# TuringLang/Bijectors.jl

Measured on NVIDIA H100. Metric: samples/sec: with_logabsdet_jacobian through 8-layer Planar flow, D=128, higher is better.
Workload: dtype f32

## Files before the change

bijectors.jl_b200/csrc/b2b_chain_v1.cu:

```cuda
#include "b2b_chain_v1_prog.cuh"

namespace b2b {

template <int D, int TPC, int CPT, int NW>
__global__ void __launch_bounds__(NW * 32, 1)
    chain_v1_kernel(const __grid_constant__ B2BChainParams P, const __grid_constant__ V1Extra E,
                    const __grid_constant__ CUtensorMap map_x, const __grid_constant__ CUtensorMap map_y) {
  const InterpProg<D, TPC, CPT> prog{P};
  v1_run<D, TPC, CPT, NW>(P, E, map_x, map_y, prog);
}

typedef void (*v1_kernel_t)(const B2BChainParams, const V1Extra, const CUtensorMap, const CUtensorMap);

struct V1Plan : V1Geom {
  v1_kernel_t kernel;
  int shape;
};

static int plan_v1(B2BChainParams& p, V1Plan& plan) {
  const int D = p.D;
  if (!(D == 32 || D == 64 || D == 128 || D == 256)) return B2B_EUNSUPPORTED;
  if (v1_check_io(p) != 0) return B2B_EUNSUPPORTED;
  int off = 0;
  for (int l = 0; l < p.L; ++l) {
    const int k = p.layers[l].kind;
    if (k == B2B_PERMUTE || k == B2B_COUPLING_AFFINE) return B2B_EUNSUPPORTED;
    p.soff[l] = off;
    off += (b2b_layer_smem_floats(p.layers[l], D) + 3) & ~3;
  }
  p.scratch_off = -1;
  bool per_row = false;
  for (int l = 0; l < p.L; ++l) per_row |= p.layers[l].kind == B2B_RQS || p.layers[l].kind == B2B_STACKED_EW;
  static const int cfg = getenv("B2B_V1_CFG") ? atoi(getenv("B2B_V1_CFG")) : 0;
  int nw, tpc, cpt = 1;
  if (D == 256) { plan.kernel = chain_v1_kernel<256, 4, 1, 12>; nw = 12; tpc = 4; }
  else if (D == 128) {
    if (cfg == 2218 && !per_row) { plan.kernel = chain_v1_kernel<128, 2, 2, 8>; nw = 8; tpc = 2; cpt = 2; }
    else if (cfg == 2112 || per_row) { plan.kernel = chain_v1_kernel<128, 2, 1, 12>; nw = 12; tpc = 2; }
    else { plan.kernel = chain_v1_kernel<128, 1, 1, 8>; nw = 8; tpc = 1; }
  }
  else if (D == 64) {
    if (cfg == 1128 && !per_row) { plan.kernel = chain_v1_kernel<64, 1, 2, 8>; nw = 8; tpc = 1; cpt = 2; }
    else { plan.kernel = chain_v1_kernel<64, 1, 1, 12>; nw = 12; tpc = 1; }
  }
  else { plan.kernel = chain_v1_kernel<32, 1, 1, 16>; nw = 16; tpc = 1; }
  plan.shape = D * 10000 + tpc * 1000 + cpt * 100 + nw;
  return v1_geometry(D, p.N, nw, (32 / tpc) * cpt, (size_t)off, plan);
}

}

int b2b_v1_plan(B2BChainParams& p, b2b::V1Geom& g, int* shape) {
  b2b::V1Plan plan;
  const int rc = b2b::plan_v1(p, plan);
  if (rc != 0) return rc;
  g = plan;
  *shape = plan.shape;
  return 0;
}

int b2b_chain_grid_size_v1(const B2BChainParams& p) {
  B2BChainParams q = p;
  b2b::V1Plan plan;
  if (b2b::plan_v1(q, plan) != 0) return 0;
  return plan.grid;
}

int b2b_launch_chain_v1(const B2BChainParams& p, cudaStream_t stream) {
  using namespace b2b;
  B2BChainParams q = p;
  V1Plan plan;
  const int rc = plan_v1(q, plan);
  if (rc != 0) return rc;
  CUtensorMap mx, my;
  if (!make_maps(q, plan.cols, &mx, &my, &plan.extra.tma3d)) return B2B_EUNSUPPORTED;
  cudaError_t e = cudaFuncSetAttribute(plan.kernel, cudaFuncAttributeMaxDynamicSharedMemorySize, (int)plan.smem);
  if (e != cudaSuccess) return (int)e;
  plan.kernel<<<plan.grid, plan.nw * 32, plan.smem, stream>>>(q, plan.extra, mx, my);
  return (int)cudaGetLastError();
}
```

bijectors.jl_b200/csrc/b2b_planar_const.cu:

```cuda
#include "b2b_planar_common.cuh"

namespace b2b {

template <int D>
struct PlanarHP {
  float v[2 * HP_MAX_L * D + 2 * HP_MAX_L];
};

template <int D>
struct ArgSrc {
  static constexpr bool kDerive = false;
  const PlanarHP<D>& H;
  int invmask;
  __device__ __forceinline__ bool inv(int l) const { return (invmask >> l) & 1; }
};

struct DevSrc {
  static constexpr bool kDerive = true;
  int invmask;
  __device__ __forceinline__ bool inv(int l) const { return (invmask >> l) & 1; }
};

template <int D, int DIR, bool MVN, class Src>
struct PlanarProg {
// ... 40 lines not shown
        acc[(i & 1) * 2 + 0] = b2b_ffma2(make_float2(w.x, w.y), x[0][2 * i], acc[(i & 1) * 2 + 0]);
        acc[(i & 1) * 2 + 1] = b2b_ffma2(make_float2(w.z, w.w), x[0][2 * i + 1], acc[(i & 1) * 2 + 1]);
      }
      const float2 s = b2b_fadd2(b2b_fadd2(acc[0], acc[1]), b2b_fadd2(acc[2], acc[3]));
      const float wz = s.x + s.y;
      const float cc_ = cb[l], bb = cb[L + l];
      float t, s2;
      if (DIR == 0 || (DIR == 2 && !src.inv(l))) {
        tanh_sech2(wz + bb, t, s2);
        lj[0] += log1pf(cc_ * s2);
      } else {
        if constexpr (TAB) find_alpha_tab(wz, cc_, bb, tab + l * PT_FLOATS, t, s2);
        else find_alpha_ts(wz, cc_, bb, t, s2);
        lj[0] -= log1pf(cc_ * s2);
        t = -t;
      }
      const float2 t2 = make_float2(t, t);
#pragma unroll
      for (int i = 0; i < D / 4; ++i) {
        const float4 u = u4[i];
        x[0][2 * i] = b2b_ffma2(make_float2(u.x, u.y), t2, x[0][2 * i]);
        x[0][2 * i + 1] = b2b_ffma2(make_float2(u.z, u.w), t2, x[0][2 * i + 1]);
      }
    }
    if (MVN) mvnormal_apply<D, 1, 1>(x, ctx, params + mvn_off(), lj);
  }
};

template <int D, int NW, int DIR>
__global__ void __launch_bounds__(NW * 32, 1)
    planar_arg_kernel(const __grid_constant__ B2BChainParams P, const __grid_constant__ V1Extra E,
                      const __grid_constant__ CUtensorMap map_x, const __grid_constant__ CUtensorMap map_y,
                      const __grid_constant__ PlanarHP<D> H, const int L, const int invmask) {
  const PlanarProg<D, DIR, false, ArgSrc<D>> prog{{H, invmask}, P, L};
  v1_run<D, 1, 1, NW>(P, E, map_x, map_y, prog);
}

template <int D, int NW, int DIR, bool MVN>
__global__ void __launch_bounds__(NW * 32, 1)
    planar_dev_kernel(const __grid_constant__ B2BChainParams P, const __grid_constant__ V1Extra E,
                      const __grid_constant__ CUtensorMap map_x, const __grid_constant__ CUtensorMap map_y,
                      const int L, const int invmask) {
  const PlanarProg<D, DIR, MVN, DevSrc> prog{{invmask}, P, L};
  v1_run<D, 1, 1, NW>(P, E, map_x, map_y, prog);
}

template <int D, int NW, int DIR>
static int launch_arg(const B2BChainParams& q, const V1Geom& g, const CUtensorMap& mx, const CUtensorMap& my, int L,
                      const float* packed, int invmask, cudaStream_t stream) {
  static PlanarHP<D> H;
  static std::mutex mu;
  std::lock_guard<std::mutex> lock(mu);
  memcpy(H.v, packed, sizeof(float) * (size_t)(2 * L * D + 2 * L));
  auto kernel = planar_arg_kernel<D, NW, DIR>;
  cudaError_t e = cudaFuncSetAttribute(kernel, cudaFuncAttributeMaxDynamicSharedMemorySize, (int)g.smem);
  if (e != cudaSuccess) return (int)e;
  kernel<<<g.grid, NW * 32, g.smem, stream>>>(q, g.extra, mx, my, H, L, invmask);
  return (int)cudaGetLastError();
}

template <int D, int NW, int DIR, bool MVN = false>
static int launch_dev(const B2BChainParams& q, const V1Geom& g, const CUtensorMap& mx, const CUtensorMap& my, int L,
                      int invmask, cudaStream_t stream) {
  auto kernel = planar_dev_kernel<D, NW, DIR, MVN>;
  cudaError_t e = cudaFuncSetAttribute(kernel, cudaFuncAttributeMaxDynamicSharedMemorySize, (int)g.smem);
  if (e != cudaSuccess) return (int)e;
  kernel<<<g.grid, NW * 32, g.smem, stream>>>(q, g.extra, mx, my, L, invmask);
  return (int)cudaGetLastError();
}

template <int D, int NW>
static int dispatch(int L, const B2BChainParams& q, const V1Geom& g, const CUtensorMap& mx, const CUtensorMap& my,
                    const float* packed, int invmask, bool mvn, cudaStream_t stream) {
  const int all = (1 << L) - 1;
  const int dir = (invmask & all) == 0 ? 0 : ((invmask & all) == all ? 1 : 2);
  if (packed) {
    if (dir == 0) return launch_arg<D, NW, 0>(q, g, mx, my, L, packed, invmask, stream);
    if (dir == 1) return launch_arg<D, NW, 1>(q, g, mx, my, L, packed, invmask, stream);
    return launch_arg<D, NW, 2>(q, g, mx, my, L, packed, invmask, stream);
  }
  if (mvn) {
    if (dir == 1) return launch_dev<D, NW, 1, true>(q, g, mx, my, L, invmask, stream);
    return B2B_EUNSUPPORTED;
  }
  if (dir == 0) return launch_dev<D, NW, 0>(q, g, mx, my, L, invmask, stream);
  if (dir == 1) return launch_dev<D, NW, 1>(q, g, mx, my, L, invmask, stream);
  return launch_dev<D, NW, 2>(q, g, mx, my, L, invmask, stream);
}

static int launch_planar(const B2BChainParams& p, int L, const float* packed, int invmask, bool mvn,
                                  cudaStream_t stream) {
  B2BChainParams q = p;
  q.scratch_off = -1;
  if (!(q.D == 32 || q.D == 64 || q.D == 128) || L < 1 || L > HP_MAX_L) return B2B_EUNSUPPORTED;
  if (v1_check_io(q) != 0) return B2B_EUNSUPPORTED;
  V1Geom g;
  const size_t pf = (size_t)((2 * L * q.D + 2 * L + 3) & ~3) + (mvn ? 2 * q.D + 4 : 0) +
                    ((!packed && invmask != 0) ? (size_t)L * PT_FLOATS : 0);
  const int rc = v1_geometry(q.D, q.N, hp_warps(q.D), 32, pf, g);
  if (rc != 0) return rc;
  CUtensorMap mx, my;
  if (!make_maps(q, g.cols, &mx, &my, &g.extra.tma3d)) return B2B_EUNSUPPORTED;
  if (q.D == 128) return dispatch<128, 8>(L, q, g, mx, my, packed, invmask, mvn, stream);
  if (q.D == 64) return dispatch<64, 12>(L, q, g, mx, my, packed, invmask, mvn, stream);
  return dispatch<32, 16>(L, q, g, mx, my, packed, invmask, mvn, stream);
}

}

int b2b_planar_const_grid_size(const B2BChainParams& p) {
  using namespace b2b;
  if (!(p.D == 32 || p.D == 64 || p.D == 128)) return 0;
  V1Geom g;
  if (v1_geometry(p.D, p.N, hp_warps(p.D), 32, 0, g) != 0) return 0;
  return g.grid;
}

int b2b_launch_planar_hostparams(const B2BChainParams& p, int L, const float* packed, int invmask,
                                 cudaStream_t stream) {
  return b2b::launch_planar(p, L, packed, invmask, false, stream);
}
// ... 25 lines not shown
```

bijectors.jl_b200/csrc/b2b_planar_vjp.cu:

```cuda
#include "b2b_planar_common.cuh"

namespace b2b {

template <int L>
struct VjpState {
  float t[L], s2[L];
};

template <int D, int L, int DIR>
struct PlanarVjpProg {
  using State = VjpState<L>;
  const B2BChainParams& P;
  int nreal;
  float* scal;
  long long N;
  __device__ __forceinline__ void stage(float* params, int warp, int lane, int nw) const {
    planar_derive_smem<D>(P, nreal, L, params, warp, lane, nw);
  }
  __device__ __forceinline__ void phase1(float2 (&x)[1][D / 2], const ColCtx<D, 1>&, const float* params,
                                         State& st) const {
#pragma unroll
    for (int l = 0; l < L; ++l) {
      const float4* w4 = reinterpret_cast<const float4*>(params + l * D);
      const float4* u4 = reinterpret_cast<const float4*>(params + L * D + l * D);
// ... 361 lines not shown
      }
      if (dir) uhb = -uhb;
    }
    const float s = block_sum_256(w * u, sh);
    const float q = block_sum_256(w * w, sh);
    const float uw = block_sum_256(uhb * w, sh);
    const float kk = (softplus(-s) - 1.0f) / q;
    const float sig_s = 1.0f / (1.0f + expf(-s)), sig_ms = 1.0f / (1.0f + expf(s));
    const float dk_ds = -sig_ms / q, dk_dq = -kk / q;
    const float cbar = dir ? -S[l * Lp + l] - gc[l] : gc[l];
    if (i < D) {
      ubar[l * D + i] = fmaf(fmaf(uw, dk_ds, cbar * sig_s), w, uhb);
      wbar[l * D + i] = wdir + kk * uhb + uw * fmaf(dk_ds, u, dk_dq * 2.0f * w) + cbar * sig_s * u;
    }
    if (i == 0) bbar[l] = gb[l];
  }
}

}

namespace b2b {

static inline size_t vjp_align(size_t v) { return (v + 255) & ~(size_t)255; }
constexpr int VJP_PG_GRID = 592;
constexpr int VJP_SS_GRID = 296;

struct VjpWs {
  float *scal, *pg_partials, *A, *ss_partials, *SS, *packed;
  size_t bytes;
};

static VjpWs vjp_carve(char* base, int Lp, int D, long long N) {
  VjpWs w;
  size_t off = 0;
  auto take = [&](size_t nfloats) {
    float* p = base ? reinterpret_cast<float*>(base + off) : nullptr;
    off += vjp_align(nfloats * sizeof(float));
    return p;
  };
  w.scal = take((size_t)N * 3 * Lp);
  w.pg_partials = take((size_t)VJP_PG_GRID * 2 * Lp * D);
  w.A = take((size_t)2 * Lp * D);
  w.ss_partials = take((size_t)VJP_SS_GRID * (Lp * Lp + 2 * Lp));
  w.SS = take((size_t)Lp * Lp + 2 * Lp);
  w.packed = take((size_t)2 * Lp * D + 2 * Lp);
  w.bytes = off + 256;
  return w;
}

template <int D, int L, int NW>
static int launch_vjp_main(int dir, const B2BChainParams& q, const V1Geom& g, const CUtensorMap& mx, const CUtensorMap& myb,
                           const CUtensorMap& mxb, float* scal, int nreal, cudaStream_t stream) {
  auto kernel = dir ? planar_vjp_kernel<D, L, NW, 1> : planar_vjp_kernel<D, L, NW, 0>;
  cudaError_t e = cudaFuncSetAttribute(kernel, cudaFuncAttributeMaxDynamicSharedMemorySize, (int)g.smem);
  if (e != cudaSuccess) return (int)e;
  kernel<<<g.grid, NW * 32, g.smem, stream>>>(q, g.extra, mx, myb, mxb, scal, nreal);
  return (int)cudaGetLastError();
}

template <int D, int NW>
static int dispatch_vjp_main(int dir, int L, const B2BChainParams& q, const V1Geom& g, const CUtensorMap& mx,
                             const CUtensorMap& myb, const CUtensorMap& mxb, float* scal, int nreal,
                             cudaStream_t stream) {
  switch (L) {
    case 1: return launch_vjp_main<D, 1, NW>(dir, q, g, mx, myb, mxb, scal, nreal, stream);
    case 2: return launch_vjp_main<D, 2, NW>(dir, q, g, mx, myb, mxb, scal, nreal, stream);
    case 4: return launch_vjp_main<D, 4, NW>(dir, q, g, mx, myb, mxb, scal, nreal, stream);
    case 8: return launch_vjp_main<D, 8, NW>(dir, q, g, mx, myb, mxb, scal, nreal, stream);
    default: return B2B_EUNSUPPORTED;
  }
}

template <int D, int L>
static int launch_pgrad_L(const float* x, const float* yb, const float* scal, long long N, long long ldx,
                          long long ldyb, float* partials, cudaStream_t stream) {
  static const int force_reg = getenv("B2B_PGRAD") && atoi(getenv("B2B_PGRAD")) == 1;
  const bool dense = ldx == D && ldyb == D && !((reinterpret_cast<uintptr_t>(x) | reinterpret_cast<uintptr_t>(yb) |
                                                 reinterpret_cast<uintptr_t>(scal)) & 15);
  if (dense && !force_reg) {
    auto kernel = planar_pgrad_bulk_kernel<D, L>;
    const int smem = PGB_STAGES * (2 * PGB_CH * D * 4 + PGB_CH * 3 * L * 4);
    cudaError_t e = cudaFuncSetAttribute(kernel, cudaFuncAttributeMaxDynamicSharedMemorySize, smem);
    if (e != cudaSuccess) return (int)e;
    kernel<<<VJP_PG_GRID, PG_THREADS, smem, stream>>>(x, yb, scal, N, partials);
  } else {
    planar_pgrad_kernel<D, L><<<VJP_PG_GRID, PG_THREADS, 0, stream>>>(x, yb, scal, N, ldx, ldyb, partials);
  }
  return (int)cudaGetLastError();
}

template <int D>
static int launch_pgrad(int L, const float* x, const float* yb, const float* scal, long long N, long long ldx,
                        long long ldyb, float* partials, cudaStream_t stream) {
  switch (L) {
    case 1: return launch_pgrad_L<D, 1>(x, yb, scal, N, ldx, ldyb, partials, stream);
    case 2: return launch_pgrad_L<D, 2>(x, yb, scal, N, ldx, ldyb, partials, stream);
    case 4: return launch_pgrad_L<D, 4>(x, yb, scal, N, ldx, ldyb, partials, stream);
    case 8: return launch_pgrad_L<D, 8>(x, yb, scal, N, ldx, ldyb, partials, stream);
    default: return B2B_EUNSUPPORTED;
  }
}

static int launch_sstat(int L, const float* scal, long long N, float* partials, cudaStream_t stream) {
  switch (L) {
    case 1: planar_sstat_kernel<1><<<VJP_SS_GRID, SS_THREADS, 0, stream>>>(scal, N, partials); break;
    case 2: planar_sstat_kernel<2><<<VJP_SS_GRID, SS_THREADS, 0, stream>>>(scal, N, partials); break;
    case 4: planar_sstat_kernel<4><<<VJP_SS_GRID, SS_THREADS, 0, stream>>>(scal, N, partials); break;
    case 8: planar_sstat_kernel<8><<<VJP_SS_GRID, SS_THREADS, 0, stream>>>(scal, N, partials); break;
    default: return B2B_EUNSUPPORTED;
  }
// ... 82 lines not shown
```

bijectors.jl_b200/csrc/b2b_radial_unrolled.cu:

```cuda
#include "b2b_v1_pipeline.cuh"

namespace b2b {

template <int D, int L, bool INV>
struct RadialProg {
  using State = V1NoState;
  const B2BChainParams& P;
  static constexpr int STRIDE = D + 4;
  __device__ __forceinline__ void stage(float* params, int warp, int lane, int nw) const {
    for (int l = warp; l < L; l += nw) stage_layer(P.layers[l], params + l * STRIDE, D, D, lane);
  }
  __device__ __forceinline__ void apply(float2 (&x)[1][D / 2], const ColCtx<D, 1>& ctx, const float* params,
                                        float (&lj)[1]) const {
#pragma unroll
    for (int l = 0; l < L; ++l) radial_apply<D, 1, 1>(x, ctx, params + l * STRIDE, INV, lj);
  }
};

template <int D, int L, int NW, bool INV>
__global__ void __launch_bounds__(NW * 32, 1)
    radial_unrolled_kernel(const __grid_constant__ B2BChainParams P, const __grid_constant__ V1Extra E,
                           const __grid_constant__ CUtensorMap map_x, const __grid_constant__ CUtensorMap map_y) {
  const RadialProg<D, L, INV> prog{P};
  v1_run<D, 1, 1, NW>(P, E, map_x, map_y, prog);
}

template <int D, int L, int NW>
static int launch_radial(const B2BChainParams& q, bool inv, cudaStream_t stream) {
  V1Geom g;
  const int rc = v1_geometry(D, q.N, NW, 32, (size_t)L * (D + 4), g);
  if (rc != 0) return rc;
  CUtensorMap mx, my;
  if (!make_maps(q, g.cols, &mx, &my, &g.extra.tma3d)) return B2B_EUNSUPPORTED;
  (void)inv;
  auto kernel = radial_unrolled_kernel<D, L, NW, true>;
  cudaError_t e = cudaFuncSetAttribute(kernel, cudaFuncAttributeMaxDynamicSharedMemorySize, (int)g.smem);
  if (e != cudaSuccess) return (int)e;
  kernel<<<g.grid, NW * 32, g.smem, stream>>>(q, g.extra, mx, my);
  return (int)cudaGetLastError();
}

template <int D, int NW>
static int dispatch_radial(const B2BChainParams& q, bool inv, cudaStream_t stream) {
  switch (q.L) {
    case 1: return launch_radial<D, 1, NW>(q, inv, stream);
    case 2: return launch_radial<D, 2, NW>(q, inv, stream);
    case 3: return launch_radial<D, 3, NW>(q, inv, stream);
    case 4: return launch_radial<D, 4, NW>(q, inv, stream);
    case 5: return launch_radial<D, 5, NW>(q, inv, stream);
    case 6: return launch_radial<D, 6, NW>(q, inv, stream);
    case 7: return launch_radial<D, 7, NW>(q, inv, stream);
    case 8: return launch_radial<D, 8, NW>(q, inv, stream);
    default: return B2B_EUNSUPPORTED;
  }
}

}

int b2b_radial_unrolled_applicable(const B2BChainParams& p) {
  if (p.L < 1 || p.L > 8 || !(p.D == 32 || p.D == 64 || p.D == 128)) return 0;
  for (int l = 0; l < p.L; ++l)
    if (p.layers[l].kind != B2B_RADIAL || !p.layers[l].inverse) return 0;
  return b2b::v1_check_io(p) == 0;
}

int b2b_launch_radial_unrolled(const B2BChainParams& p, cudaStream_t stream) {
  using namespace b2b;
  if (!b2b_radial_unrolled_applicable(p)) return B2B_EUNSUPPORTED;
  B2BChainParams q = p;
  q.scratch_off = -1;
  const bool inv = p.layers[0].inverse != 0;
  if (q.D == 128) return dispatch_radial<128, 8>(q, inv, stream);
  if (q.D == 64) return dispatch_radial<64, 12>(q, inv, stream);
  return dispatch_radial<32, 16>(q, inv, stream);
}
```

bijectors.jl_b200/csrc/b2b_rqs_unrolled.cu:

```cuda
#include "b2b_v1_pipeline.cuh"

namespace b2b {

constexpr int RQS_REC = 12;

__host__ __device__ constexpr int rqs2_steps(int K1) {
  int s = 0;
  while ((1 << s) < K1 - 1) ++s;
  return s;
}
__host__ __device__ constexpr bool rqs2_supported(int K1) { return K1 >= 2 && K1 <= 33; }
__host__ __device__ constexpr int rqs2_row_floats(int K1) { return (K1 + 1) * RQS_REC; }

__device__ __forceinline__ float rcp_ftz(float x) {
  float r;
  asm("rcp.approx.ftz.f32 %0, %1;" : "=f"(r) : "f"(x));
  return r;
}
__device__ __forceinline__ float lg2_ftz(float x) {
  float r;
  asm("lg2.approx.ftz.f32 %0, %1;" : "=f"(r) : "f"(x));
  return r;
}
__device__ __forceinline__ float sqrt_ftz(float x) {
// ... 102 lines not shown
  const float rden = rcp_ftz(fmaf(ds, xo, sl));
  const float inner = fmaf(sl + sl, xo, fmaf(d_k1 * xi, xi, d_k * omx * omx));
  const float q = sl * rden;
  const float arg = q * q * inner;
  if (!INV) res = fmaf(dy * fmaf(sl * xi, xi, d_k * xo), rden, h_k);
  out = outside ? v : res;
  lg = lg2_ftz(outside ? 1.0f : arg);
}

template <int D, int K1, bool INV>
struct RqsProg {
  using State = V1NoState;
  const B2BChainParams& P;
  __device__ __forceinline__ void stage(float* params, int warp, int lane, int nw) const {
    stage_rqs_records<K1, INV>(P.layers[0], params, D, warp * 32 + lane, nw * 32);
  }
  __device__ __forceinline__ void apply(float2 (&x)[1][D / 2], const ColCtx<D, 1>&, const float* params,
                                        float (&lj)[1]) const {
    constexpr int RF = rqs2_row_floats(K1);
    float acc[4] = {0.f, 0.f, 0.f, 0.f};
    uint32_t pbase = smem_u32(params);
    asm volatile("" : "+r"(pbase));
#pragma unroll
    for (int i = 0; i < D / 2; ++i) {
      float o, l1;
      rqs2_element<K1, INV>(pbase + (2 * i) * RF * 4, x[0][i].x, o, l1);
      x[0][i].x = o;
      acc[(2 * i) & 3] += l1;
      rqs2_element<K1, INV>(pbase + (2 * i + 1) * RF * 4, x[0][i].y, o, l1);
      x[0][i].y = o;
      acc[(2 * i + 1) & 3] += l1;
    }
    const float s = ((acc[0] + acc[1]) + (acc[2] + acc[3])) * 0.6931471805599453f;
    lj[0] += INV ? -s : s;
  }
};

template <int D, int K1, int NW, bool INV>
__global__ void __launch_bounds__(NW * 32, 1)
    rqs_unrolled_kernel(const __grid_constant__ B2BChainParams P, const __grid_constant__ V1Extra E,
                        const __grid_constant__ CUtensorMap map_x, const __grid_constant__ CUtensorMap map_y) {
  const RqsProg<D, K1, INV> prog{P};
  v1_run<D, 1, 1, NW>(P, E, map_x, map_y, prog);
}

template <int D, int K1, int NW>
static int launch_rqs(const B2BChainParams& q, cudaStream_t stream) {
  V1Geom g;
  const int rc = v1_geometry(D, q.N, NW, 32, (size_t)D * rqs2_row_floats(K1), g);
  if (rc != 0) return rc;
  CUtensorMap mx, my;
  if (!make_maps(q, g.cols, &mx, &my, &g.extra.tma3d)) return B2B_EUNSUPPORTED;
  auto kernel = q.layers[0].inverse ? rqs_unrolled_kernel<D, K1, NW, true> : rqs_unrolled_kernel<D, K1, NW, false>;
  cudaError_t e = cudaFuncSetAttribute(kernel, cudaFuncAttributeMaxDynamicSharedMemorySize, (int)g.smem);
  if (e != cudaSuccess) return (int)e;
  kernel<<<g.grid, NW * 32, g.smem, stream>>>(q, g.extra, mx, my);
  return (int)cudaGetLastError();
}

template <int D, int NW>
static int dispatch_rqs(const B2BChainParams& q, cudaStream_t stream) {
  const int K1r = q.layers[0].n0;
  if (K1r < 2 || K1r > 33) return B2B_EUNSUPPORTED;
  if (K1r <= 5) return launch_rqs<D, 5, NW>(q, stream);
  if (K1r <= 9) return launch_rqs<D, 9, NW>(q, stream);
  if (K1r <= 17) return launch_rqs<D, 17, NW>(q, stream);
  return launch_rqs<D, 33, NW>(q, stream);
}

}

int b2b_rqs_unrolled_applicable(const B2BChainParams& p) {
  return p.L == 1 && p.layers[0].kind == B2B_RQS && b2b::rqs2_supported(p.layers[0].n0) && (p.D == 32 || p.D == 64) &&
         b2b::v1_check_io(p) == 0;
}

int b2b_rqs_unrolled_warps(int D) { return D == 64 ? 12 : 16; }

int b2b_launch_rqs_unrolled(const B2BChainParams& p, cudaStream_t stream) {
  using namespace b2b;
  if (!b2b_rqs_unrolled_applicable(p)) return B2B_EUNSUPPORTED;
  B2BChainParams q = p;
  q.scratch_off = -1;
  if (q.D == 64) return dispatch_rqs<64, 12>(q, stream);
  return dispatch_rqs<32, 16>(q, stream);
}
```

bijectors.jl_b200/csrc/b2b_sample.cu:

```cuda
#include "b2b_chain_v1_prog.cuh"

int b2b_v1_plan(B2BChainParams& p, b2b::V1Geom& g, int* shape);

namespace b2b {

__global__ void __launch_bounds__(256) randn_kernel(float* __restrict__ z, const V1Gen g, int D, long long N, long long ld) {
  const int Dc = (D + 3) >> 2;
  const long long total = N * Dc;
  const bool vec = (D % 4 == 0) && (ld % 4 == 0) && ((reinterpret_cast<uintptr_t>(z) & 15) == 0);
  for (long long i = (long long)blockIdx.x * blockDim.x + threadIdx.x; i < total; i += (long long)gridDim.x * blockDim.x) {
    const long long n = i / Dc;
    const int k = (int)(i - n * Dc);
    float4 v = philox_normal4(g, g.col0 + n, k);
    float e[4] = {v.x, v.y, v.z, v.w};
#pragma unroll
    for (int q = 0; q < 4; ++q) {
      const int r = 4 * k + q;
      if (r < D) {
        if (g.sigma) e[q] *= g.sigma[r];
        if (g.mu) e[q] += g.mu[r];
      }
    }
    float* dst = z + n * ld + 4 * k;
    if (vec) {
      *reinterpret_cast<float4*>(dst) = make_float4(e[0], e[1], e[2], e[3]);
    } else {
#pragma unroll
      for (int q = 0; q < 4; ++q)
        if (4 * k + q < D) dst[q] = e[q];
    }
  }
}

template <int D, int TPC, int CPT, int NW>
__global__ void __launch_bounds__(NW * 32, 1)
    chain_sample_kernel(const __grid_constant__ B2BChainParams P, const __grid_constant__ V1Extra E,
                        const __grid_constant__ CUtensorMap map_y, const __grid_constant__ V1Gen G) {
  const InterpProg<D, TPC, CPT> prog{P};
  v1_run<D, TPC, CPT, NW, InterpProg<D, TPC, CPT>, 1, true>(P, E, map_y, map_y, prog, nullptr, &G);
}

template <int D, int TPC, int CPT, int NW>
static int launch_sample(const B2BChainParams& q, const V1Geom& g, const CUtensorMap& my, const V1Gen& gen, cudaStream_t stream) {
  auto kernel = chain_sample_kernel<D, TPC, CPT, NW>;
  cudaError_t e = cudaFuncSetAttribute(kernel, cudaFuncAttributeMaxDynamicSharedMemorySize, (int)g.smem);
  if (e != cudaSuccess) return (int)e;
  kernel<<<g.grid, NW * 32, g.smem, stream>>>(q, g.extra, my, gen);
  return (int)cudaGetLastError();
}

}

static bool fusable_kind(int kind) {
  return kind == B2B_PLANAR || kind == B2B_RADIAL || kind == B2B_RQS || kind == B2B_BATCHNORM || kind == B2B_STACKED_EW;
}

extern "C" int b2b_randn_f32(float* z, const float* mu, const float* sigma, uint64_t seed, uint64_t offset,
                             int64_t column_offset, int32_t D, int64_t N, int64_t ld, void* stream_) {
  using namespace b2b;
  if (D < 1 || N < 0 || ld < D) return B2B_EINVAL;
  if (N == 0) return B2B_OK;
  if (!z) return B2B_EINVAL;
  V1Gen g{seed, offset, column_offset, mu, sigma};
  const long long total = N * ((D + 3) / 4);
  long long blocks = (total + 255) / 256;
  if (blocks > 132 * 16) blocks = 132 * 16;
  randn_kernel<<<(int)blocks, 256, 0, static_cast<cudaStream_t>(stream_)>>>(z, g, D, N, ld);
  return (int)cudaGetLastError();
}

extern "C" int b2b_chain_sample_f32(const b2b_layer_desc* layers, int32_t L, const float* mu, const float* sigma,
                                    uint64_t seed, uint64_t offset, int64_t column_offset, float* y, float* logjac,
                                    int32_t D, int64_t N, int64_t ldy, void* workspace, size_t workspace_bytes,
                                    void* stream_) {
  using namespace b2b;
  cudaStream_t stream = static_cast<cudaStream_t>(stream_);
  if (L < 0 || L > B2B_MAX_CHAIN || (L > 0 && !layers) || D < 1 || N < 0 || ldy < D) return B2B_EINVAL;
  if (N == 0) return B2B_OK;
  if (!y) return B2B_EINVAL;
  if (L == 0) {
    if (logjac) {
      cudaError_t e = cudaMemsetAsync(logjac, 0, (size_t)N * sizeof(float), stream);
      if (e != cudaSuccess) return (int)e;
    }
    return b2b_randn_f32(y, mu, sigma, seed, offset, column_offset, D, N, ldy, stream_);
  }
  bool fused = (D % 4 == 0) && (!mu || (reinterpret_cast<uintptr_t>(mu) & 15) == 0) &&
               (!sigma || (reinterpret_cast<uintptr_t>(sigma) & 15) == 0);
  for (int l = 0; l < L && fused; ++l) fused = fusable_kind(layers[l].kind);
  if (fused) {
    B2BChainParams p;
    memset(&p, 0, sizeof(p));
    p.x = y;
    p.y = y;
    p.logjac = logjac;
    p.N = N;
    p.ldx = ldy;
    p.ldy = ldy;
    p.D = D;
    p.L = L;
    for (int l = 0; l < L; ++l) p.layers[l] = layers[l];
// ... 22 lines not shown
```

bijectors.jl_b200/csrc/b2b_v1_pipeline.cuh:

```cuda
#pragma once
#include <cuda.h>
#include <cuda_runtime.h>

#include <cstdlib>
#include <mutex>

#include "b2b_device.cuh"

namespace b2b {

__device__ __forceinline__ uint32_t smem_u32(const void* p) {
  return static_cast<uint32_t>(__cvta_generic_to_shared(p));
}
__device__ __forceinline__ void mbar_init(uint32_t bar, uint32_t count) {
  asm volatile("mbarrier.init.shared::cta.b64 [%0], %1;" ::"r"(bar), "r"(count));
}
__device__ __forceinline__ void mbar_expect_tx(uint32_t bar, uint32_t bytes) {
  asm volatile("mbarrier.arrive.expect_tx.shared::cta.b64 _, [%0], %1;" ::"r"(bar), "r"(bytes) : "memory");
}
__device__ __forceinline__ void mbar_wait(uint32_t bar, uint32_t parity) {
  asm volatile(
      "{\n"
      ".reg .pred P1;\n"
      "B2B_WAIT:\n"
      "mbarrier.try_wait.parity.shared::cta.b64 P1, [%0], %1;\n"
      "@P1 bra B2B_DONE;\n"
      "bra B2B_WAIT;\n"
      "B2B_DONE:\n"
      "}\n" ::"r"(bar),
      "r"(parity)
      : "memory");
}
__device__ __forceinline__ void tma_load_2d(uint32_t dst, const CUtensorMap* map, int c0, int c1, uint32_t bar) {
  asm volatile(
      "cp.async.bulk.tensor.2d.shared::cluster.global.mbarrier::complete_tx::bytes [%0], [%1, {%2, %3}], [%4];" ::"r"(dst),
      "l"(reinterpret_cast<uint64_t>(map)), "r"(c0), "r"(c1), "r"(bar)
      : "memory");
}
__device__ __forceinline__ void tma_store_2d(const CUtensorMap* map, int c0, int c1, uint32_t src, uint64_t pol) {
  asm volatile("cp.async.bulk.tensor.2d.global.shared::cta.bulk_group.L2::cache_hint [%0, {%1, %2}], [%3], %4;" ::"l"(
                   reinterpret_cast<uint64_t>(map)),
               "r"(c0), "r"(c1), "r"(src), "l"(pol)
               : "memory");
}
__device__ __forceinline__ void tma_load_3d(uint32_t dst, const CUtensorMap* map, int c0, int c1, int c2, uint32_t bar) {
  asm volatile(
      "cp.async.bulk.tensor.3d.shared::cluster.global.mbarrier::complete_tx::bytes [%0], [%1, {%2, %3, %4}], [%5];" ::"r"(dst),
      "l"(reinterpret_cast<uint64_t>(map)), "r"(c0), "r"(c1), "r"(c2), "r"(bar)
      : "memory");
}
__device__ __forceinline__ void tma_store_3d(const CUtensorMap* map, int c0, int c1, int c2, uint32_t src, uint64_t pol) {
  asm volatile("cp.async.bulk.tensor.3d.global.shared::cta.bulk_group.L2::cache_hint [%0, {%1, %2, %3}], [%4], %5;" ::"l"(
                   reinterpret_cast<uint64_t>(map)),
               "r"(c0), "r"(c1), "r"(c2), "r"(src), "l"(pol)
               : "memory");
}
__device__ __forceinline__ uint64_t l2_evict_first() {
  uint64_t p;
  asm volatile("createpolicy.fractional.L2::evict_first.b64 %0, 1.0;" : "=l"(p));
  return p;
}
__device__ __forceinline__ void mbar_arrive(uint32_t bar) {
  asm volatile("mbarrier.arrive.shared::cta.b64 _, [%0];" ::"r"(bar) : "memory");
}
__device__ __forceinline__ void bulk_load_1d(uint32_t dst, const void* src, uint32_t bytes, uint32_t bar) {
  asm volatile("cp.async.bulk.shared::cluster.global.mbarrier::complete_tx::bytes [%0], [%1], %2, [%3];" ::"r"(dst),
               "l"(reinterpret_cast<uint64_t>(src)), "r"(bytes), "r"(bar)
               : "memory");
}
__device__ __forceinline__ void tma_commit() { asm volatile("cp.async.bulk.commit_group;" ::: "memory"); }
__device__ __forceinline__ void tma_wait_read0() { asm volatile("cp.async.bulk.wait_group.read 0;" ::: "memory"); }
__device__ __forceinline__ void tma_wait_all0() { asm volatile("cp.async.bulk.wait_group 0;" ::: "memory"); }
__device__ __forceinline__ void fence_proxy_async() { asm volatile("fence.proxy.async.shared::cta;" ::: "memory"); }
__device__ __forceinline__ void fence_mbar_init() { asm volatile("fence.mbarrier_init.release.cluster;" ::: "memory"); }
__device__ __forceinline__ void flag_store_release(int* p, int v) {
  asm volatile("st.release.cta.shared::cta.s32 [%0], %1;" ::"r"(smem_u32(p)), "r"(v) : "memory");
}
__device__ __forceinline__ int flag_load_acquire(const int* p) {
  int v;
  asm volatile("ld.acquire.cta.shared::cta.s32 %0, [%1];" : "=r"(v) : "r"(smem_u32(p)) : "memory");
  return v;
}

struct V1Extra {
  int n_in;
  int param_off;
  int bar_off;
  int nwarps;
  int tma3d;
  long long tiles;
};

template <int D, int TPC>
struct ColCtx {
  static constexpr int EPT = D / TPC;
  static constexpr int NQT = EPT / 32;
  int h, rot;
  __device__ __forceinline__ int prm(int ql, int r) const { return (h * NQT + ql) * 8 + (r ^ rot); }
  __device__ __forceinline__ int row(int ql, int r, int e) const { return prm(ql, r) * 4 + e; }
};

template <int TPC>
__device__ __forceinline__ float part_sum(float v) {
#pragma unroll
  for (int o = 1; o < TPC; o <<= 1) v += __shfl_xor_sync(0xffffffffu, v, o);
  return v;
}

#define B2B_FOR_SLOTS                        \
  _Pragma("unroll") for (int ql = 0; ql < C::NQT; ++ql) _Pragma("unroll") for (int r = 0; r < 8; ++r)
#define B2B_FOR_COLS _Pragma("unroll") for (int cc = 0; cc < CPT; ++cc)

template <int D, int TPC, int CPT>
__device__ __forceinline__ void radial_apply(float2 (&x)[CPT][D / TPC / 2], const ColCtx<D, TPC>& c, const float* sp,
                                             bool inverse, float (&lj)[CPT]) {
  using C = ColCtx<D, TPC>;
  const float4* z4 = reinterpret_cast<const float4*>(sp);
  const float alpha = sp[D], bhat = sp[D + 1], apb = sp[D + 2];
  const float2 m1 = make_float2(-1.f, -1.f);
  float2 acc[CPT][4];
  B2B_FOR_COLS {
#pragma unroll
    for (int i = 0; i < 4; ++i) acc[cc][i] = make_float2(0.f, 0.f);
  }
  B2B_FOR_SLOTS {
    const float4 z0 = z4[c.prm(ql, r)];
    const int i = (ql * 8 + r) * 2;
// ... 95 lines not shown
  const float u2 = fmaf(__uint2float_rn(b), 2.3283064365386963e-10f, 1.1641532182693481e-10f);
  const float r = sqrtf(-1.3862943611198906f * __log2f(u1));
  const float ang = 6.283185307179586f * u2 - 3.141592653589793f;
  z0 = -r * __cosf(ang);
  z1 = -r * __sinf(ang);
}

__device__ __forceinline__ float4 philox_normal4(const V1Gen& g, long long n, int k) {
  uint32_t o[4];
  philox4x32_10((uint32_t)n, (uint32_t)((unsigned long long)n >> 32), (uint32_t)k, (uint32_t)g.offset, (uint32_t)g.seed,
                (uint32_t)(g.seed >> 32), o);
  float4 z;
  box_muller(o[0], o[1], z.x, z.y);
  box_muller(o[2], o[3], z.z, z.w);
  return z;
}

struct V1NoState {};

template <int D, int TPC, int CPT, int NW, class Prog, int NIN = 1, bool GEN = false>
__device__ __forceinline__ void v1_run(const B2BChainParams& P, const V1Extra& E, const CUtensorMap& map_x,
                                       const CUtensorMap& map_y, const Prog& prog,
                                       const CUtensorMap* map_x2 = nullptr, const V1Gen* gen = nullptr) {
  using C = ColCtx<D, TPC>;
  constexpr int NQ = D / 32;
  constexpr int LPC = 32 / TPC;
  constexpr int COLS = LPC * CPT;
  constexpr int BOX_BYTES = COLS * 128;
  constexpr int TILE_BYTES = NQ * BOX_BYTES;
  constexpr int SLOT_BYTES = NIN * TILE_BYTES;
  extern __shared__ unsigned char smem_dyn[];
  unsigned char* smem_raw = smem_dyn + ((1024u - (smem_u32(smem_dyn) & 1023u)) & 1023u);
  unsigned char* in_base = smem_raw;
  unsigned char* out_base = smem_raw + (size_t)E.n_in * SLOT_BYTES;
  float* params = reinterpret_cast<float*>(smem_raw + E.param_off);
  uint64_t* bars = reinterpret_cast<uint64_t*>(smem_raw + E.bar_off);
  int* armed = reinterpret_cast<int*>(bars + 8);

  const int lane = threadIdx.x & 31, warp = __shfl_sync(0xffffffffu, (int)(threadIdx.x >> 5), 0);
  auto load_tile = [&](uint32_t dst, int col0, uint32_t bar) {
    if (E.tma3d) {
      tma_load_3d(dst, &map_x, 0, col0, 0, bar);
      if (NIN == 2) tma_load_3d(dst + TILE_BYTES, map_x2, 0, col0, 0, bar);
    } else {
#pragma unroll
      for (int q = 0; q < NQ; ++q) tma_load_2d(dst + q * BOX_BYTES, &map_x, q * 32, col0, bar);
      if (NIN == 2) {
#pragma unroll
        for (int q = 0; q < NQ; ++q) tma_load_2d(dst + TILE_BYTES + q * BOX_BYTES, map_x2, q * 32, col0, bar);
      }
    }
  };
  const long long my_tiles = (E.tiles - blockIdx.x + gridDim.x - 1) / gridDim.x;
  if (threadIdx.x == 0 && !GEN) {
    for (int i = 0; i < E.n_in; ++i) mbar_init(smem_u32(&bars[i]), 1);
    fence_mbar_init();
    for (int j = 0; j < E.n_in && j < my_tiles; ++j) {
      const uint32_t bar = smem_u32(&bars[j]);
      mbar_expect_tx(bar, SLOT_BYTES);
      const long long tile = blockIdx.x + (long long)j * gridDim.x;
      load_tile(smem_u32(in_base + (size_t)j * SLOT_BYTES), (int)(tile * COLS), bar);
      flag_store_release(&armed[j], j);
    }
  }
  prog.stage(params, warp, lane, NW);
  __syncthreads();

  C ctx;
  const int t = lane / TPC;
  ctx.h = lane % TPC;
  ctx.rot = ctx.h * (8 / TPC);
  unsigned char* my_out = out_base + (size_t)warp * TILE_BYTES;
  const int sw = (((t & 7) ^ ctx.rot) & 7) * 16;
  const int line = t * 128 + ctx.h * C::NQT * BOX_BYTES;
  double dsum = 0.0;
  bool store_pending = false;

  for (long long j = warp; j < my_tiles; j += NW) {
    const int buf = (int)(j % E.n_in);
    const uint32_t parity = (uint32_t)((j / E.n_in) & 1);
    const long long tile = blockIdx.x + j * gridDim.x;
    const long long col = tile * COLS + t;
    if constexpr (!GEN) {
      while (flag_load_acquire(&armed[buf]) != (int)j) __nanosleep(20);
      mbar_wait(smem_u32(&bars[buf]), parity);
    }

    float2 x[CPT][C::EPT / 2];
    auto load_fragment = [&](const unsigned char* src) {
      B2B_FOR_COLS {
        B2B_FOR_SLOTS {
          const float4 v =
              *reinterpret_cast<const float4*>(src + cc * (LPC * 128) + ql * BOX_BYTES + ((r * 16) ^ sw));
          x[cc][(ql * 8 + r) * 2] = make_float2(v.x, v.y);
          x[cc][(ql * 8 + r) * 2 + 1] = make_float2(v.z, v.w);
        }
      }
    };
    if constexpr (GEN) {
      B2B_FOR_COLS {
        const long long n = gen->col0 + col + cc * LPC;
        B2B_FOR_SLOTS {
          const int row0 = ctx.row(ql, r, 0);
          float4 z = philox_normal4(*gen, n, row0 >> 2);
          if (gen->sigma) {
            const float4 sg = __ldg(reinterpret_cast<const float4*>(gen->sigma + row0));
            z = make_float4(z.x * sg.x, z.y * sg.y, z.z * sg.z, z.w * sg.w);
          }
          if (gen->mu) {
            const float4 m = __ldg(reinterpret_cast<const float4*>(gen->mu + row0));
            z = make_float4(z.x + m.x, z.y + m.y, z.z + m.z, z.w + m.w);
          }
          x[cc][(ql * 8 + r) * 2] = make_float2(z.x, z.y);
          x[cc][(ql * 8 + r) * 2 + 1] = make_float2(z.z, z.w);
        }
      }
    } else {
      load_fragment(in_base + (size_t)buf * SLOT_BYTES + line);
    }
    typename Prog::State st;
    if constexpr (NIN == 2) {
      prog.phase1(x, ctx, params, st);
      load_fragment(in_base + (size_t)buf * SLOT_BYTES + TILE_BYTES + line);
    }
    if constexpr (!GEN) fence_proxy_async();
    __syncwarp();
    if (!GEN && lane == 0 && j + E.n_in < my_tiles) {
      const uint32_t bar = smem_u32(&bars[buf]);
      mbar_expect_tx(bar, SLOT_BYTES);
      const long long nt = blockIdx.x + (j + E.n_in) * gridDim.x;
      load_tile(smem_u32(in_base + (size_t)buf * SLOT_BYTES), (int)(nt * COLS), bar);
      flag_store_release(&armed[buf], (int)(j + E.n_in));
    }

    float lj[CPT];
    B2B_FOR_COLS {
      const long long cl = col + cc * LPC;
      lj[cc] = (P.accumulate && P.logjac && cl < P.N) ? P.logjac[cl] : 0.0f;
    }
    if constexpr (NIN == 2) prog.apply(x, ctx, params, lj, st, col);
    else prog.apply(x, ctx, params, lj);

    if (P.y) {
      if (store_pending) {
        if (lane == 0) tma_wait_read0();
        __syncwarp();
      }
      unsigned char* dst = my_out + line;
      B2B_FOR_COLS {
        B2B_FOR_SLOTS {
          const float2 a = x[cc][(ql * 8 + r) * 2], b = x[cc][(ql * 8 + r) * 2 + 1];
          *reinterpret_cast<float4*>(dst + cc * (LPC * 128) + ql * BOX_BYTES + ((r * 16) ^ sw)) =
              make_float4(a.x, a.y, b.x, b.y);
        }
      }
      fence_proxy_async();
      __syncwarp();
      if (lane == 0) {
        const uint64_t pol = l2_evict_first();
        if (E.tma3d) {
          tma_store_3d(&map_y, 0, (int)(tile * COLS), 0, smem_u32(my_out), pol);
        } else {
#pragma unroll
          for (int q = 0; q < NQ; ++q)
            tma_store_2d(&map_y, q * 32, (int)(tile * COLS), smem_u32(my_out + q * BOX_BYTES), pol);
        }
        tma_commit();
      }
      store_pending = true;
    }
    if (ctx.h == 0) {
      B2B_FOR_COLS {
        const long long cl = col + cc * LPC;
        if (cl < P.N) {
          if (P.logjac && !(P.accumulate & 2)) P.logjac[cl] = lj[cc];
          dsum += (double)lj[cc];
        }
      }
    }
  }
  if (lane == 0 && store_pending) tma_wait_all0();

  if (P.partials) {
    __shared__ double red[32];
#pragma unroll
// ... 21 lines not shown
    if (cudaGetDriverEntryPoint("cuTensorMapEncodeTiled", &p, cudaEnableDefault, &q) == cudaSuccess &&
        q == cudaDriverEntryPointSuccess)
      fn = reinterpret_cast<encode_tiled_fn>(p);
  });
  return fn;
}

static inline bool make_map(CUtensorMap* m, const float* base, int D, long long N, long long ld, int cols, bool three_d) {
  encode_tiled_fn enc = get_encode();
  if (!enc) return false;
  const cuuint32_t estr[3] = {1, 1, 1};
  if (three_d) {
    const cuuint64_t dims[3] = {32, (cuuint64_t)N, (cuuint64_t)(D / 32)};
    const cuuint64_t strides[2] = {(cuuint64_t)ld * sizeof(float), 128};
    const cuuint32_t box[3] = {32, (cuuint32_t)cols, (cuuint32_t)(D / 32)};
    return enc(m, CU_TENSOR_MAP_DATA_TYPE_FLOAT32, 3, const_cast<float*>(base), dims, strides, box, estr,
               CU_TENSOR_MAP_INTERLEAVE_NONE, CU_TENSOR_MAP_SWIZZLE_128B, CU_TENSOR_MAP_L2_PROMOTION_L2_128B,
               CU_TENSOR_MAP_FLOAT_OOB_FILL_NONE) == CUDA_SUCCESS;
  }
  const cuuint64_t dims[2] = {(cuuint64_t)D, (cuuint64_t)N};
  const cuuint64_t strides[1] = {(cuuint64_t)ld * sizeof(float)};
  const cuuint32_t box[2] = {32, (cuuint32_t)cols};
  return enc(m, CU_TENSOR_MAP_DATA_TYPE_FLOAT32, 2, const_cast<float*>(base), dims, strides, box, estr,
             CU_TENSOR_MAP_INTERLEAVE_NONE, CU_TENSOR_MAP_SWIZZLE_128B, CU_TENSOR_MAP_L2_PROMOTION_L2_128B,
             CU_TENSOR_MAP_FLOAT_OOB_FILL_NONE) == CUDA_SUCCESS;
}

static inline bool make_maps(const B2BChainParams& q, int cols, CUtensorMap* mx, CUtensorMap* my, int* tma3d) {
  static const int force2d = getenv("B2B_V1_TMA") && atoi(getenv("B2B_V1_TMA")) == 2;
  for (int three_d = force2d ? 0 : 1; three_d >= 0; --three_d) {
    if (three_d && q.D == 32) continue;
    bool ok = make_map(mx, q.x, q.D, q.N, q.ldx, cols, three_d != 0);
    if (ok && q.y) ok = make_map(my, q.y, q.D, q.N, q.ldy, cols, three_d != 0);
    if (ok) {
      if (!q.y) *my = *mx;
      *tma3d = three_d;
      return true;
    }
  }
  return false;
}

struct V1Geom {
  int nw, grid, cols;
  size_t smem;
  V1Extra extra;
};

static inline int v1_check_io(const B2BChainParams& p) {
  if (p.N >= (1ll << 31) - 64) return B2B_EUNSUPPORTED;
  if ((p.ldx % 4) || (reinterpret_cast<uintptr_t>(p.x) & 15)) return B2B_EUNSUPPORTED;
  if (p.y && ((p.ldy % 4) || (reinterpret_cast<uintptr_t>(p.y) & 15))) return B2B_EUNSUPPORTED;
  return 0;
}

static inline int v1_geometry(int D, long long N, int nw, int cols, size_t param_floats, V1Geom& g,
                              int in_tiles = 1) {
  const int tile_bytes = D * 4 * cols;
  const size_t param_bytes = param_floats * sizeof(float);
  const size_t budget = 225 * 1024;
  const size_t fixed = (size_t)nw * tile_bytes + ((param_bytes + 15) & ~(size_t)15) + 16 * sizeof(uint64_t) + 1024;
  const size_t slot_bytes = (size_t)in_tiles * tile_bytes;
  if (fixed + 2 * slot_bytes > budget) return B2B_EUNSUPPORTED;
  int n_in = (int)((budget - fixed) / slot_bytes);
  if (n_in > 8) n_in = 8;
  g.nw = nw;
  g.cols = cols;
  g.extra.n_in = n_in;
  g.extra.nwarps = nw;
  g.extra.tma3d = 0;
  g.extra.param_off = n_in * (int)slot_bytes + nw * tile_bytes;
  g.extra.bar_off = g.extra.param_off + (int)((param_bytes + 15) & ~(size_t)15);
  g.extra.tiles = (N + cols - 1) / cols;
  g.smem = (size_t)g.extra.bar_off + 16 * sizeof(uint64_t) + 1024;
  int dev = 0, sms = 0;
  cudaGetDevice(&dev);
  cudaDeviceGetAttribute(&sms, cudaDevAttrMultiProcessorCount, dev);
  long long grid = sms;
  const long long want = (g.extra.tiles + nw - 1) / nw;
  if (grid > want) grid = want;
  if (grid < 1) grid = 1;
  g.grid = (int)grid;
  return 0;
}

}
```

Baseline: 2.584 billion.

## Add programmatic dependent launch and cache host launch attributes for v1 kernels

Routes all v1 kernel launches through a shared helper that launches with cudaLaunchKernelEx and the programmatic stream serialization attribute. Kernels prefetch tensor maps and initialize barriers before griddepcontrol.wait, then signal dependents once their last input tile load is issued. The helper also caches the dynamic shared memory attribute per kernel and device, and caches the SM count, to cut per-launch host calls. The overlap relies on the correctness of where the wait and trigger are placed, and the map lookup adds a mutex on every launch.

```diff
diff --git a/bijectors.jl_b200/csrc/b2b_chain_v1.cu b/bijectors.jl_b200/csrc/b2b_chain_v1.cu
--- a/bijectors.jl_b200/csrc/b2b_chain_v1.cu
+++ b/bijectors.jl_b200/csrc/b2b_chain_v1.cu
@@ -74,8 +74,5 @@
   if (rc != 0) return rc;
   CUtensorMap mx, my;
   if (!make_maps(q, plan.cols, &mx, &my, &plan.extra.tma3d)) return B2B_EUNSUPPORTED;
-  cudaError_t e = cudaFuncSetAttribute(plan.kernel, cudaFuncAttributeMaxDynamicSharedMemorySize, (int)plan.smem);
-  if (e != cudaSuccess) return (int)e;
-  plan.kernel<<<plan.grid, plan.nw * 32, plan.smem, stream>>>(q, plan.extra, mx, my);
-  return (int)cudaGetLastError();
+  return launch_v1(plan.kernel, plan.grid, plan.nw * 32, plan.smem, stream, q, plan.extra, mx, my);
 }
diff --git a/bijectors.jl_b200/csrc/b2b_planar_const.cu b/bijectors.jl_b200/csrc/b2b_planar_const.cu
--- a/bijectors.jl_b200/csrc/b2b_planar_const.cu
+++ b/bijectors.jl_b200/csrc/b2b_planar_const.cu
@@ -116,21 +116,13 @@
   static std::mutex mu;
   std::lock_guard<std::mutex> lock(mu);
   memcpy(H.v, packed, sizeof(float) * (size_t)(2 * L * D + 2 * L));
-  auto kernel = planar_arg_kernel<D, NW, DIR>;
-  cudaError_t e = cudaFuncSetAttribute(kernel, cudaFuncAttributeMaxDynamicSharedMemorySize, (int)g.smem);
-  if (e != cudaSuccess) return (int)e;
-  kernel<<<g.grid, NW * 32, g.smem, stream>>>(q, g.extra, mx, my, H, L, invmask);
-  return (int)cudaGetLastError();
+  return launch_v1(planar_arg_kernel<D, NW, DIR>, g.grid, NW * 32, g.smem, stream, q, g.extra, mx, my, H, L, invmask);
 }
 
 template <int D, int NW, int DIR, bool MVN = false>
 static int launch_dev(const B2BChainParams& q, const V1Geom& g, const CUtensorMap& mx, const CUtensorMap& my, int L,
                       int invmask, cudaStream_t stream) {
-  auto kernel = planar_dev_kernel<D, NW, DIR, MVN>;
-  cudaError_t e = cudaFuncSetAttribute(kernel, cudaFuncAttributeMaxDynamicSharedMemorySize, (int)g.smem);
-  if (e != cudaSuccess) return (int)e;
-  kernel<<<g.grid, NW * 32, g.smem, stream>>>(q, g.extra, mx, my, L, invmask);
-  return (int)cudaGetLastError();
+  return launch_v1(planar_dev_kernel<D, NW, DIR, MVN>, g.grid, NW * 32, g.smem, stream, q, g.extra, mx, my, L, invmask);
 }
 
 template <int D, int NW>
diff --git a/bijectors.jl_b200/csrc/b2b_planar_vjp.cu b/bijectors.jl_b200/csrc/b2b_planar_vjp.cu
--- a/bijectors.jl_b200/csrc/b2b_planar_vjp.cu
+++ b/bijectors.jl_b200/csrc/b2b_planar_vjp.cu
@@ -437,10 +437,7 @@
 static int launch_vjp_main(int dir, const B2BChainParams& q, const V1Geom& g, const CUtensorMap& mx, const CUtensorMap& myb,
                            const CUtensorMap& mxb, float* scal, int nreal, cudaStream_t stream) {
   auto kernel = dir ? planar_vjp_kernel<D, L, NW, 1> : planar_vjp_kernel<D, L, NW, 0>;
-  cudaError_t e = cudaFuncSetAttribute(kernel, cudaFuncAttributeMaxDynamicSharedMemorySize, (int)g.smem);
-  if (e != cudaSuccess) return (int)e;
-  kernel<<<g.grid, NW * 32, g.smem, stream>>>(q, g.extra, mx, myb, mxb, scal, nreal);
-  return (int)cudaGetLastError();
+  return launch_v1(kernel, g.grid, NW * 32, g.smem, stream, q, g.extra, mx, myb, mxb, scal, nreal);
 }
 
 template <int D, int NW>
diff --git a/bijectors.jl_b200/csrc/b2b_radial_unrolled.cu b/bijectors.jl_b200/csrc/b2b_radial_unrolled.cu
--- a/bijectors.jl_b200/csrc/b2b_radial_unrolled.cu
+++ b/bijectors.jl_b200/csrc/b2b_radial_unrolled.cu
@@ -33,11 +33,7 @@
   CUtensorMap mx, my;
   if (!make_maps(q, g.cols, &mx, &my, &g.extra.tma3d)) return B2B_EUNSUPPORTED;
   (void)inv;
-  auto kernel = radial_unrolled_kernel<D, L, NW, true>;
-  cudaError_t e = cudaFuncSetAttribute(kernel, cudaFuncAttributeMaxDynamicSharedMemorySize, (int)g.smem);
-  if (e != cudaSuccess) return (int)e;
-  kernel<<<g.grid, NW * 32, g.smem, stream>>>(q, g.extra, mx, my);
-  return (int)cudaGetLastError();
+  return launch_v1(radial_unrolled_kernel<D, L, NW, true>, g.grid, NW * 32, g.smem, stream, q, g.extra, mx, my);
 }
 
 template <int D, int NW>
diff --git a/bijectors.jl_b200/csrc/b2b_rqs_unrolled.cu b/bijectors.jl_b200/csrc/b2b_rqs_unrolled.cu
--- a/bijectors.jl_b200/csrc/b2b_rqs_unrolled.cu
+++ b/bijectors.jl_b200/csrc/b2b_rqs_unrolled.cu
@@ -178,10 +178,7 @@
   CUtensorMap mx, my;
   if (!make_maps(q, g.cols, &mx, &my, &g.extra.tma3d)) return B2B_EUNSUPPORTED;
   auto kernel = q.layers[0].inverse ? rqs_unrolled_kernel<D, K1, NW, true> : rqs_unrolled_kernel<D, K1, NW, false>;
-  cudaError_t e = cudaFuncSetAttribute(kernel, cudaFuncAttributeMaxDynamicSharedMemorySize, (int)g.smem);
-  if (e != cudaSuccess) return (int)e;
-  kernel<<<g.grid, NW * 32, g.smem, stream>>>(q, g.extra, mx, my);
-  return (int)cudaGetLastError();
+  return launch_v1(kernel, g.grid, NW * 32, g.smem, stream, q, g.extra, mx, my);
 }
 
 template <int D, int NW>
diff --git a/bijectors.jl_b200/csrc/b2b_sample.cu b/bijectors.jl_b200/csrc/b2b_sample.cu
--- a/bijectors.jl_b200/csrc/b2b_sample.cu
+++ b/bijectors.jl_b200/csrc/b2b_sample.cu
@@ -42,11 +42,7 @@
 
 template <int D, int TPC, int CPT, int NW>
 static int launch_sample(const B2BChainParams& q, const V1Geom& g, const CUtensorMap& my, const V1Gen& gen, cudaStream_t stream) {
-  auto kernel = chain_sample_kernel<D, TPC, CPT, NW>;
-  cudaError_t e = cudaFuncSetAttribute(kernel, cudaFuncAttributeMaxDynamicSharedMemorySize, (int)g.smem);
-  if (e != cudaSuccess) return (int)e;
-  kernel<<<g.grid, NW * 32, g.smem, stream>>>(q, g.extra, my, gen);
-  return (int)cudaGetLastError();
+  return launch_v1(chain_sample_kernel<D, TPC, CPT, NW>, g.grid, NW * 32, g.smem, stream, q, g.extra, my, gen);
 }
 
 }
diff --git a/bijectors.jl_b200/csrc/b2b_v1_pipeline.cuh b/bijectors.jl_b200/csrc/b2b_v1_pipeline.cuh
--- a/bijectors.jl_b200/csrc/b2b_v1_pipeline.cuh
+++ b/bijectors.jl_b200/csrc/b2b_v1_pipeline.cuh
@@ -2,8 +2,11 @@
 #include <cuda.h>
 #include <cuda_runtime.h>
 
+#include <atomic>
 #include <cstdlib>
+#include <map>
 #include <mutex>
+#include <utility>
 
 #include "b2b_device.cuh"
 
@@ -73,6 +76,11 @@
 __device__ __forceinline__ void tma_wait_all0() { asm volatile("cp.async.bulk.wait_group 0;" ::: "memory"); }
 __device__ __forceinline__ void fence_proxy_async() { asm volatile("fence.proxy.async.shared::cta;" ::: "memory"); }
 __device__ __forceinline__ void fence_mbar_init() { asm volatile("fence.mbarrier_init.release.cluster;" ::: "memory"); }
+__device__ __forceinline__ void prefetch_tensormap(const CUtensorMap* map) {
+  asm volatile("prefetch.tensormap [%0];" ::"l"(reinterpret_cast<uint64_t>(map)) : "memory");
+}
+__device__ __forceinline__ void griddep_wait() { asm volatile("griddepcontrol.wait;" ::: "memory"); }
+__device__ __forceinline__ void griddep_launch_dependents() { asm volatile("griddepcontrol.launch_dependents;" ::: "memory"); }
 __device__ __forceinline__ void flag_store_release(int* p, int v) {
   asm volatile("st.release.cta.shared::cta.s32 [%0], %1;" ::"r"(smem_u32(p)), "r"(v) : "memory");
 }
@@ -274,16 +282,27 @@
     }
   };
   const long long my_tiles = (E.tiles - blockIdx.x + gridDim.x - 1) / gridDim.x;
-  if (threadIdx.x == 0 && !GEN) {
-    for (int i = 0; i < E.n_in; ++i) mbar_init(smem_u32(&bars[i]), 1);
-    fence_mbar_init();
-    for (int j = 0; j < E.n_in && j < my_tiles; ++j) {
-      const uint32_t bar = smem_u32(&bars[j]);
-      mbar_expect_tx(bar, SLOT_BYTES);
-      const long long tile = blockIdx.x + (long long)j * gridDim.x;
-      load_tile(smem_u32(in_base + (size_t)j * SLOT_BYTES), (int)(tile * COLS), bar);
-      flag_store_release(&armed[j], j);
-    }
+  if (threadIdx.x == 0) {
+    prefetch_tensormap(&map_y);
+    if (!GEN) {
+      prefetch_tensormap(&map_x);
+      if (NIN == 2) prefetch_tensormap(map_x2);
+      for (int i = 0; i < E.n_in; ++i) mbar_init(smem_u32(&bars[i]), 1);
+      fence_mbar_init();
+    }
+  }
+  griddep_wait();
+  if (threadIdx.x == 0) {
+    if (!GEN) {
+      for (int j = 0; j < E.n_in && j < my_tiles; ++j) {
+        const uint32_t bar = smem_u32(&bars[j]);
+        mbar_expect_tx(bar, SLOT_BYTES);
+        const long long tile = blockIdx.x + (long long)j * gridDim.x;
+        load_tile(smem_u32(in_base + (size_t)j * SLOT_BYTES), (int)(tile * COLS), bar);
+        flag_store_release(&armed[j], j);
+      }
+    }
+    if (GEN || my_tiles <= E.n_in) griddep_launch_dependents();
   }
   prog.stage(params, warp, lane, NW);
   __syncthreads();
@@ -353,6 +372,7 @@
       const long long nt = blockIdx.x + (j + E.n_in) * gridDim.x;
       load_tile(smem_u32(in_base + (size_t)buf * SLOT_BYTES), (int)(nt * COLS), bar);
       flag_store_release(&armed[buf], (int)(j + E.n_in));
+      if (j + E.n_in == my_tiles - 1) griddep_launch_dependents();
     }
 
     float lj[CPT];
@@ -480,6 +500,57 @@
   if ((p.ldx % 4) || (reinterpret_cast<uintptr_t>(p.x) & 15)) return B2B_EUNSUPPORTED;
   if (p.y && ((p.ldy % 4) || (reinterpret_cast<uintptr_t>(p.y) & 15))) return B2B_EUNSUPPORTED;
   return 0;
+}
+
+constexpr int kMaxDevices = 64;
+
+static inline int device_sm_count(int dev) {
+  static std::atomic<int> cache[kMaxDevices];
+  int sms = (dev >= 0 && dev < kMaxDevices) ? cache[dev].load(std::memory_order_relaxed) : 0;
+  if (sms == 0) {
+    cudaDeviceGetAttribute(&sms, cudaDevAttrMultiProcessorCount, dev);
+    if (sms > 0 && dev >= 0 && dev < kMaxDevices) cache[dev].store(sms, std::memory_order_relaxed);
+  }
+  return sms;
+}
+
+static inline cudaError_t ensure_dynamic_smem(const void* kernel, size_t smem) {
+  static std::mutex mu;
+  static std::map<std::pair<const void*, int>, size_t> granted;
+  int dev = 0;
+  cudaError_t e = cudaGetDevice(&dev);
+  if (e != cudaSuccess) return e;
+  std::lock_guard<std::mutex> lock(mu);
+  size_t& have = granted[{kernel, dev}];
+  if (smem <= have) return cudaSuccess;
+  e = cudaFuncSetAttribute(kernel, cudaFuncAttributeMaxDynamicSharedMemorySize, (int)smem);
+  if (e == cudaSuccess) have = smem;
+  return e;
+}
+
+static inline bool pdl_enabled() {
+  static const bool on = !(getenv("B2B_PDL") && atoi(getenv("B2B_PDL")) == 0);
+  return on;
+}
+
+template <class... KArgs, class... Args>
+static int launch_v1(void (*kernel)(KArgs...), int grid, int threads, size_t smem, cudaStream_t stream,
+                     Args&&... args) {
+  cudaError_t e = ensure_dynamic_smem(reinterpret_cast<const void*>(kernel), smem);
+  if (e != cudaSuccess) return (int)e;
+  cudaLaunchAttribute attr[1];
+  attr[0].id = cudaLaunchAttributeProgrammaticStreamSerialization;
+  attr[0].val.programmaticStreamSerializationAllowed = 1;
+  cudaLaunchConfig_t cfg = {};
+  cfg.gridDim = dim3((unsigned)grid);
+  cfg.blockDim = dim3((unsigned)threads);
+  cfg.dynamicSmemBytes = smem;
+  cfg.stream = stream;
+  cfg.attrs = attr;
+  cfg.numAttrs = pdl_enabled() ? 1 : 0;
+  e = cudaLaunchKernelEx(&cfg, kernel, std::forward<Args>(args)...);
+  const cudaError_t last = cudaGetLastError();
+  return (int)(e != cudaSuccess ? e : last);
 }
 
 static inline int v1_geometry(int D, long long N, int nw, int cols, size_t param_floats, V1Geom& g,
@@ -501,10 +572,9 @@
   g.extra.bar_off = g.extra.param_off + (int)((param_bytes + 15) & ~(size_t)15);
   g.extra.tiles = (N + cols - 1) / cols;
   g.smem = (size_t)g.extra.bar_off + 16 * sizeof(uint64_t) + 1024;
-  int dev = 0, sms = 0;
+  int dev = 0;
   cudaGetDevice(&dev);
-  cudaDeviceGetAttribute(&sms, cudaDevAttrMultiProcessorCount, dev);
-  long long grid = sms;
+  long long grid = device_sm_count(dev);
   const long long want = (g.extra.tiles + nw - 1) / nw;
   if (grid > want) grid = want;
   if (grid < 1) grid = 1;
```

After: 2.628 billion (median of 6 runs). 1.7% higher.
